# LIA-DiTella/DiffUDF

Hardware: AMD Instinct MI355X
Metric: train points/sec (SIREN fwd+∇x+Eikonal loss+bwd), 256×8 net, 100k pts (higher is better)
Workload: dtype f32

## Files before the change

### diffudf_amd/_lib.py

```python
import ctypes
import os

_HERE = os.path.dirname(os.path.abspath(__file__))
LIB_PATH = os.environ.get("DUDF_LIB") or os.path.join(_HERE, "libdudf_hip.so")

LOSS_S1, LOSS_S2, LOSS_SIREN = 0, 1, 2

_ERRORS = {
    -1: "DUDF_E_BADCFG: unsupported network (kernel width in {32,64,128,256,512} — hip_ops pads narrower / unequal layers —, n_in=3, n_out=1)",
    -2: "DUDF_E_WORKSPACE: workspace too small or misaligned",
    -3: "DUDF_E_BADMODE",
    -4: "DUDF_E_UNSUPPORTED: this configuration has no HIP path; there is deliberately no CPU fallback",
}


class NetCfg(ctypes.Structure):
    _fields_ = [("n_in", ctypes.c_int32), ("n_hidden_layers", ctypes.c_int32),
                ("hidden", ctypes.c_int32), ("w0", ctypes.c_float), ("ww", ctypes.c_float)]


class DudfError(RuntimeError):
    pass


# ... 65 lines not shown
                                            ctypes.c_size_t, _P]),
    "dudf_adam_step": (ctypes.c_int, [_P, _P, _P, _P, ctypes.c_int64, ctypes.c_double, ctypes.c_double,
                                      ctypes.c_double, ctypes.c_double, ctypes.c_int64, ctypes.c_double, _P]),
    "dudf_adam_schedule": (ctypes.c_int, [_DBL, ctypes.c_int64, ctypes.c_int64, ctypes.c_double, ctypes.c_double, _P]),
    "dudf_adam_step_scheduled": (ctypes.c_int, [_P, _P, _P, _P, ctypes.c_int64, ctypes.c_double, ctypes.c_double, ctypes.c_double,
                                                _P, ctypes.c_int64, _P, ctypes.c_double, _P]),
    "dudf_sample_batch_at": (ctypes.c_int, [_P, ctypes.c_int64, _P, _P, ctypes.c_int64, ctypes.c_int64, ctypes.c_int64,
                                            ctypes.c_int64, ctypes.c_uint64, _P, ctypes.c_int, ctypes.c_int, _P, _P, _P, _P]),
    "dudf_sample_batch": (ctypes.c_int, [_P, ctypes.c_int64, _P, _P, ctypes.c_int64, ctypes.c_int64, ctypes.c_int64,
                                         ctypes.c_int64, ctypes.c_uint64, ctypes.c_uint64, ctypes.c_int, ctypes.c_int,
                                         _P, _P, _P, _P]),
    "dudf_capudf_workspace_bytes": (ctypes.c_size_t, [ctypes.c_int64]),
    "dudf_capudf_count": (ctypes.c_int, [_P, _P, ctypes.c_int64, ctypes.c_double, _P, _P, ctypes.c_size_t, _P]),
    "dudf_capudf_emit": (ctypes.c_int, [_P, _P, ctypes.c_int64, ctypes.c_double, _P, _P, _P, _P, ctypes.c_size_t, _P]),
    "dudf_profile_enable": (ctypes.c_int, [ctypes.c_int]),
    "dudf_split_mode": (ctypes.c_int, []),
    "dudf_profile_dump": (ctypes.c_int, [ctypes.c_char_p, ctypes.c_size_t]),
    "dudf_profile_clocks": (ctypes.c_int, [ctypes.c_char_p, ctypes.c_size_t]),
    "dudf_profile_products": (ctypes.c_int, [ctypes.c_char_p, ctypes.c_size_t]),
    "dudf_set_wgrad_max_workgroups": (ctypes.c_int, [ctypes.c_int]),
    "dudf_debug_read_stash": (ctypes.c_int, [_CFG, ctypes.c_int, ctypes.c_int, ctypes.c_int, ctypes.c_int64,
                                             ctypes.c_int64, _P, _P, ctypes.c_size_t, _P]),
    "dudf_debug_stash_layout": (ctypes.c_int, [_CFG, ctypes.c_int64, ctypes.c_int64, ctypes.POINTER(ctypes.c_int64)]),
    "dudf_debug_kernel_choice": (ctypes.c_int, [_CFG, ctypes.c_int64, ctypes.c_int64, ctypes.c_int, ctypes.c_int, ctypes.c_char_p, ctypes.c_size_t]),
    "dudf_stash_mode": (ctypes.c_int, [_CFG, ctypes.c_int64, ctypes.c_int64]),
    "dudf_set_option": (ctypes.c_int, [ctypes.c_char_p, ctypes.c_int]),
    "dudf_get_option": (ctypes.c_int, [ctypes.c_char_p, ctypes.POINTER(ctypes.c_int)]),
    "dudf_reset_options": (ctypes.c_int, []),
    "dudf_abi_version": (ctypes.c_int, []),
}
ABI_VERSION = 8


def load():
    global _lib
    if _lib is not None:
        return _lib
    if not os.path.exists(LIB_PATH):
        raise DudfError(f"{LIB_PATH} not found: build it with `python -c 'import __graft_entry__ as g; g.build()'` "
                        "(hipcc --offload-arch=gfx950). There is no CPU fallback for the HIP path.")
    lib = ctypes.CDLL(LIB_PATH)
    try:
        lib.dudf_abi_version.restype = ctypes.c_int
        abi = int(lib.dudf_abi_version())
    except AttributeError:
        abi = None
# ... 22 lines not shown
```

### diffudf_amd/csrc/dudf_api.hip

```cpp
#include "dudf_internal.h"
#include <stdio.h>
#include <stdlib.h>
#include <string.h>
#include <vector>

namespace {
struct ProfRec { int slot; hipEvent_t e0, e1; };
bool g_prof_on = false;
std::vector<ProfRec> g_prof_recs;
std::vector<hipEvent_t> g_prof_pool;
hipEvent_t g_prof_open[PROF_NSLOTS];
const char* kProfNames[PROF_NSLOTS] = {"pack", "sweep_fwd", "sweep_rev", "sweep_adj_fwd", "sweep_adj_rev",
                                       "wgrad_hidden", "wgrad_small", "loss_fwd", "loss_bwd", "adam", "other"};
unsigned long long* g_prof_clk = nullptr;
hipEvent_t prof_event() {
    if (!g_prof_pool.empty()) { hipEvent_t e = g_prof_pool.back(); g_prof_pool.pop_back(); return e; }
    hipEvent_t e; (void)hipEventCreate(&e); return e;
}
}

namespace { int g_products[PROF_NSLOTS] = {0}; }
void dudf_note_products(int slot, int products) { if (slot >= 0 && slot < PROF_NSLOTS) g_products[slot] = products; }

unsigned long long* dudf_prof_clk(int slot) { return (g_prof_on && g_prof_clk) ? g_prof_clk + 2 * slot : nullptr; }
// ... 803 lines not shown
    if (layer < 0 || layer >= c.lo.L || channel < 0 || channel > 3) return DUDF_E_BADCFG;
    const DudfLayout& lo = c.lo;
    const int64_t offs[8] = {lo.ws_S, lo.ws_C, lo.ws_Q, lo.ws_E, lo.ws_A, lo.ws_Z, lo.ws_R, lo.ws_ZS};
    if (which < 0 || which > 7) return DUDF_E_BADMODE;
    const bool sqaz = which == 0 || which == 2 || which == 4 || which == 5;
    const int b24 = which == 7 ? 0 : which == 1 ? ((lo.p24 & 4) ? 2 : 0) : sqaz ? ((lo.p24 & 1) ? 3 : 0) : ((lo.p24 & 2) ? 1 : 0);
    const int fxi = which == 0 ? 0 : which == 2 ? 1 : which == 4 ? 2 : 3;
    return dudf_launch_read_stash(lo, c.ws + offs[which], layer, channel, out, c.st, which == 1, b24,
                                  b24 == 3 ? c.ws + lo.ws_fx[fxi] : nullptr);
}

int dudf_debug_stash_layout(const dudf_net_cfg* cfg, int64_t n, int64_t n_hess, int64_t* out) {
    DudfLayout lo;
    int rc = dudf_make_layout(cfg, n, n_hess, &lo);
    if (rc) return rc;
    if (!out) return DUDF_E_BADCFG;
    const int64_t offs[8] = {lo.ws_S, lo.ws_C, lo.ws_Q, lo.ws_E, lo.ws_A, lo.ws_Z, lo.ws_R, lo.ws_ZS};
    for (int i = 0; i < 8; ++i) out[i] = offs[i] * (int64_t)sizeof(float);
    out[8] = lo.np * 16;
    out[9] = lo.stash_layer * (int64_t)sizeof(float);
    return 0;
}

int dudf_debug_kernel_choice(const dudf_net_cfg* cfg, int64_t n, int64_t n_hess, int which, int flags, char* name, size_t name_len) {
    DudfLayout lo;
    int rc = dudf_make_layout(cfg, n, n_hess, &lo, (flags & 16) != 0);
    if (rc) return rc;
    if (!name || name_len == 0) return DUDF_E_BADCFG;
    name[0] = 0;
    SweepChoice c;
    if (which == DUDF_CHOICE_WGRAD) {
        c = dudf_choose_wgrad(WgradRequest{lo.H, lo.L, lo.p24 & 1, lo.np}, dudf_options());
    } else {
        const SweepRequest r = {which & 15, lo.H, lo.L, flags & 1, (flags >> 1) & 1, (flags >> 2) & 1, (flags >> 3) & 1, split_mask(), lo.p24,
                                lo.ws_ebound != lo.ws_amax, lo.ws_zbound != lo.ws_amax};
        c = (which & DUDF_CHOICE_PAIR) ? dudf_choose_pair(r, dudf_options()) : dudf_choose_sweep(r, dudf_options());
    }
    if (c.status == 0 && dudf_choice_name(c, name, name_len) >= (int)name_len) return DUDF_E_WORKSPACE;
    return c.status;
}

int dudf_stash_mode(const dudf_net_cfg* cfg, int64_t n, int64_t n_hess) {
    DudfLayout lo;
    if (dudf_make_layout(cfg, n, n_hess, &lo)) return -1;
    return lo.p24;
}
// ... 3 lines not shown
```

### diffudf_amd/csrc/dudf_internal.h

```cpp
#pragma once
#include <hip/hip_runtime.h>
#include <stdint.h>
#include <stdlib.h>
#include "../../include/dudf_hip.h"
#include "dudf_variants.h"

typedef float f32x4 __attribute__((ext_vector_type(4)));
typedef float f32x16 __attribute__((ext_vector_type(16)));
typedef float f32x2 __attribute__((ext_vector_type(2)));
typedef unsigned u32x4 __attribute__((ext_vector_type(4)));
typedef __bf16 bf16x8 __attribute__((ext_vector_type(8)));
typedef __bf16 bf16x2 __attribute__((ext_vector_type(2)));
typedef _Float16 f16x8 __attribute__((ext_vector_type(8)));
typedef _Float16 f16x2 __attribute__((ext_vector_type(2)));

__device__ __forceinline__ unsigned cvt_pk(f32x2 v) {
    return __builtin_bit_cast(unsigned, __builtin_convertvector(v, bf16x2));
}
__device__ __forceinline__ f32x2 unpack(unsigned p) {
    return f32x2{__builtin_bit_cast(float, p << 16), __builtin_bit_cast(float, p & 0xffff0000u)};
}

#define DUDF_TILE_PTS 64
#define DUDF_COL_PAD 128
#define DUDF_NACC 16

struct DudfLayout {
    int H, L;
    float rho;
    int p24;
    float w0;
    int64_t n, n_h;
    int64_t ncol_h, ncol_n;
    int64_t ncols;
    int64_t np;
    int64_t off_w1, off_b1, off_hid, hid_stride, off_wo, off_bo, n_theta;
    int64_t ws_w1b, ws_b1s, ws_w1t16, ws_wt, ws_wimg, ws_wimg16, ws_wsc, ws_amax, ws_ebound, ws_zbound, ws_x4, ws_y, ws_g, ws_ybar, ws_gbar;
    int64_t ws_S, ws_C, ws_ZS, ws_Q, ws_R, ws_E, ws_A, ws_Z, ws_acc;
    int64_t ws_fx[4];
    int64_t stash_layer;
    size_t total_bytes;
};

DudfOptions dudf_options();

static inline int dudf_make_layout(const dudf_net_cfg* cfg, int64_t n, int64_t n_h, DudfLayout* lo, int query_only = 0) {
    if (!cfg || cfg->n_in != 3 || cfg->n_hidden_layers < 1) return DUDF_E_BADCFG;
    const int H = cfg->hidden, L = cfg->n_hidden_layers;
    if (!(H == 32 || H == 64 || H == 128 || H == 256 || H == 512)) return DUDF_E_BADCFG;
    if (n < 0 || n_h < 0 || n_h > n) return DUDF_E_BADCFG;
    if (!(cfg->w0 > 0.f) || cfg->ww < 0.f) return DUDF_E_BADCFG;
    const float ww = cfg->ww > 0.f ? cfg->ww : cfg->w0;
    lo->H = H; lo->L = L; lo->w0 = ww; lo->rho = cfg->w0 / ww;
    lo->n = n; lo->n_h = n_h;
    lo->p24 = query_only ? 0 : dudf_stash_p24_enabled(H, L, dudf_options());
    auto pad = [](int64_t c) { return (c + DUDF_COL_PAD - 1) / DUDF_COL_PAD * DUDF_COL_PAD; };
    lo->ncol_h = pad(4 * n_h);
    lo->ncol_n = pad(n - n_h);
    lo->np = lo->ncol_h + lo->ncol_n;
    if (lo->np == 0) { lo->ncol_n = DUDF_COL_PAD; lo->np = DUDF_COL_PAD; }
    lo->ncols = lo->np;
    if (lo->np % 2048 == 0) lo->np += 32;
    if (lo->np * 1024 >= (1ll << 32)) lo->p24 = 0;
// ... 11 lines not shown
    lo->ws_wimg16 = take((int64_t)(L - 1) * H * H * 2);
    lo->ws_wsc = take(2 * (int64_t)(L > 1 ? L - 1 : 1));
    lo->ws_amax = take(4 * (int64_t)L);
    lo->ws_ebound = query_only ? lo->ws_amax : take((int64_t)L * lo->np);
    lo->ws_zbound = (n_h == 0) ? lo->ws_amax : take((int64_t)L * lo->ncol_h);
    lo->ws_x4 = take(4 * lo->np);
    lo->ws_y = take(lo->np); lo->ws_g = take(4 * lo->np);
    lo->ws_ybar = take(lo->np); lo->ws_gbar = take(4 * lo->np);
    lo->stash_layer = (int64_t)H * lo->np;
    const int64_t stash = (int64_t)L * lo->stash_layer;
    const int64_t stash_b = (lo->p24 & 1) ? stash / 4 * 3 : stash;
    const int64_t stash_r = (lo->p24 & 2) ? stash / 4 * 3 : stash;
    const int64_t stash_c = (lo->p24 & 4) ? stash / 4 * 3 : stash;
    lo->ws_S = take(stash_b); lo->ws_C = take(stash_c);
    lo->ws_ZS = n_h > 0 ? take(stash) : lo->ws_S;
    if (query_only) {
        lo->ws_Q = lo->ws_R = lo->ws_E = lo->ws_A = lo->ws_Z = lo->ws_S;
    } else {
        lo->ws_Q = take(stash_b); lo->ws_R = take(stash_r); lo->ws_E = take(stash_r); lo->ws_A = take(stash_b);
        lo->ws_Z = take(stash_b);
    }
    for (int i = 0; i < 4; ++i) lo->ws_fx[i] = (lo->p24 & 1) ? take((int64_t)L * lo->np) : lo->ws_amax;
    lo->ws_acc = take(2 * DUDF_NACC);
    lo->total_bytes = (size_t)o * sizeof(float);
    return 0;
}

#if defined(__HIP_DEVICE_COMPILE__)
#define DUDF_NO_PK __attribute__((target("no-packed-fp32-ops")))
#else
#define DUDF_NO_PK
#endif

struct SweepArgs {
    const float* theta; const float* w1b; const float* b1s; const float* w1t16; const float* wt;
    const char* wimg_f; const char* wimg_t;
    const char* wimg16_f; const char* wimg16_t;
    const float* wsc;
    unsigned* amax;
    float* ebound;
    float* zbound;
    int64_t nch;
    unsigned long long* clk;
    int split;
    const float* x4;
    float* y; float* g;
// ... 105 lines not shown
```

### diffudf_amd/csrc/dudf_prep.hip

```cpp
#include "dudf_sweep16.h"

namespace {

template <int H>
__device__ __forceinline__ void pack_bf16_body(const float* __restrict__ theta, char* __restrict__ img_f,
                                               char* __restrict__ img_t, int nhid, int64_t off_hid,
                                               int64_t hid_stride, int64_t block, int64_t nblocks) {
    using G = GeoB<H>;
    const int64_t total = (int64_t)2 * nhid * G::NKB * G::NT * 64;
    for (int64_t idx = block * 256 + threadIdx.x; idx < total; idx += nblocks * 256) {
        int64_t v = idx;
        const int lane = (int)(v & 63); v >>= 6;
        const int T = (int)(v % G::NT); v /= G::NT;
        const int kb = (int)(v % G::NKB); v /= G::NKB;
        const int j = (int)(v % nhid); v /= nhid;
        const int dir = (int)v;
        const int m = lane & 15, g = lane >> 4;
        const int row = 16 * T + m;
        const float* W = theta + off_hid + (int64_t)j * hid_stride;
        f32x4 e0, e1;
#pragma unroll
        for (int e = 0; e < 4; ++e) {
            const int f0 = 32 * kb + 4 * g + e, f1 = f0 + 16;
            e0[e] = dir == 0 ? W[(int64_t)row * H + f0] : W[(int64_t)f0 * H + row];
// ... 53 lines not shown
            e1[e] = sc * (dir == 0 ? W[(int64_t)row * H + f1] : W[(int64_t)f1 * H + row]);
        }
        u32x4 h, l;
        split8h(e0, e1, h, l);
        char* base = (dir == 0 ? img_f : img_t) + (size_t)j * G::IMGB + (size_t)kb * G::CHUNKB + (size_t)T * 2 * G::FRAG + lane * 16;
        *reinterpret_cast<u32x4*>(base) = h;
        *reinterpret_cast<u32x4*>(base + G::FRAG) = l;
    }
}
template <int H>
__global__ __launch_bounds__(256) void pack_f16_kernel(const float* __restrict__ theta, char* __restrict__ img_f,
                                                       char* __restrict__ img_t, float* __restrict__ wsc, int nhid,
                                                       int64_t off_hid, int64_t hid_stride) {
    pack_f16_body<H>(theta, img_f, img_t, wsc, nhid, off_hid, hid_stride, blockIdx.y, blockIdx.x, gridDim.x);
}

struct PrepArgs {
    const float* theta; const float* x;
    float *w1b, *b1s, *w1t16, *wt, *x4, *wsc;
    float rho;
    char *img16_f, *img16_t, *img_f, *img_t;
    unsigned* zero; int nzero;
    unsigned* zero2; int nzero2;
    int L, nsub;
    int64_t off_hid, hid_stride, n, n_h, ncol_h, np;
    int nb_f16, nb_bf16, nb_x4, nb_thin, nb_wt;
};
template <int H>
__global__ __launch_bounds__(256) void prep_kernel(PrepArgs a) {
    int b = blockIdx.x;
    const int nhid = a.L - 1;
    if (b < a.nb_f16) { pack_f16_body<H>(a.theta, a.img16_f, a.img16_t, a.wsc, nhid, a.off_hid, a.hid_stride, b / a.nsub, b % a.nsub, a.nsub); return; }
    b -= a.nb_f16;
    if (b < a.nb_bf16) { pack_bf16_body<H>(a.theta, a.img_f, a.img_t, nhid, a.off_hid, a.hid_stride, b, a.nb_bf16); return; }
    b -= a.nb_bf16;
    if (b < a.nb_x4) {
        for (int64_t c = (int64_t)b * 256 + threadIdx.x; c < a.np; c += (int64_t)a.nb_x4 * 256) {
            f32x4 v = {0, 0, 0, 0};
            if (c < a.ncol_h) {
                const int64_t p = c >> 2; const int ch = (int)(c & 3);
                if (p < a.n_h) {
                    if (ch == 0) v = f32x4{a.x[p * 3], a.x[p * 3 + 1], a.x[p * 3 + 2], 1.f};
                    else v[ch - 1] = 1.f;
                }
            } else {
                const int64_t p = a.n_h + (c - a.ncol_h);
// ... 4 lines not shown
        return;
    }
    b -= a.nb_x4;
    if (b < a.nb_thin) {
        const int n_thin = 16 * H > a.L * H ? 16 * H : a.L * H;
        for (int gid = b * 256 + threadIdx.x; gid < n_thin; gid += a.nb_thin * 256) {
            if (gid < 4 * H) {
                const int f = gid / 4, k = gid % 4;
                a.w1b[gid] = a.rho * (k < 3 ? a.theta[f * 3 + k] : a.theta[3 * H + f]);
                if (k == 3) a.b1s[f] = a.rho * a.theta[3 * H + f];
            }
            if (gid >= H && gid < a.L * H) {
                const int layer = gid / H, f = gid % H;
                a.b1s[gid] = a.theta[a.off_hid + (int64_t)(layer - 1) * a.hid_stride + (int64_t)H * H + f];
            }
            if (gid < 16 * H) {
                const int r = gid / H, f = gid % H;
                a.w1t16[gid] = r < 3 ? a.rho * a.theta[f * 3 + r] : 0.f;
            }
        }
        if (b == 0) {
            for (int i = threadIdx.x; i < a.nzero; i += 256) a.zero[i] = 0u;
            for (int i = threadIdx.x; i < a.nzero2; i += 256) a.zero2[i] = 0u;
        }
        return;
    }
    b -= a.nb_thin;
    {
        const int64_t n_wt = (int64_t)nhid * H * H;
        for (int64_t gid = (int64_t)b * 256 + threadIdx.x; gid < n_wt; gid += (int64_t)a.nb_wt * 256) {
            const int64_t j = gid / ((int64_t)H * H), rem = gid % ((int64_t)H * H);
            const int i = (int)(rem / H), o = (int)(rem % H);
            a.wt[gid] = a.theta[a.off_hid + j * a.hid_stride + (int64_t)o * H + i];
        }
    }
}

template <int H>
int pack_b(const DudfLayout& lo, const float* theta, float* ws, hipStream_t st) {
    using G = GeoB<H>;
    char* img_f = reinterpret_cast<char*>(ws + lo.ws_wimg);
    char* img_t = img_f + (size_t)(lo.L - 1) * G::IMGB;
    const int64_t total = (int64_t)2 * (lo.L - 1) * G::NKB * G::NT * 64;
    hipLaunchKernelGGL(pack_bf16_kernel<H>, dim3((unsigned)((total + 255) / 256)), dim3(256), 0, st, theta, img_f, img_t,
                       lo.L - 1, lo.off_hid, lo.hid_stride);
    if (dudf_split_fp16()) {
        using G1 = GeoB<H, 1>;
        char* i16_f = reinterpret_cast<char*>(ws + lo.ws_wimg16);
        char* i16_t = i16_f + (size_t)(lo.L - 1) * G1::IMGB;
        hipLaunchKernelGGL(pack_f16_kernel<H>, dim3(H >= 256 ? 16 : 4, lo.L - 1), dim3(256), 0, st, theta, i16_f, i16_t,
                           ws + lo.ws_wsc, lo.L - 1, lo.off_hid, lo.hid_stride);
    }
    return (int)hipGetLastError();
}

template <int H>
int prep_b(const DudfLayout& lo, const float* theta, const float* x, float* ws, int need, hipStream_t st) {
    PrepArgs a;
    a.theta = theta; a.x = x;
    a.w1b = ws + lo.ws_w1b; a.b1s = ws + lo.ws_b1s; a.rho = lo.rho; a.w1t16 = ws + lo.ws_w1t16; a.wt = ws + lo.ws_wt; a.x4 = ws + lo.ws_x4; a.wsc = ws + lo.ws_wsc;
    a.img_f = reinterpret_cast<char*>(ws + lo.ws_wimg); a.img_t = a.img_f + (size_t)(lo.L - 1) * GeoB<H>::IMGB;
    a.img16_f = reinterpret_cast<char*>(ws + lo.ws_wimg16); a.img16_t = a.img16_f + (size_t)(lo.L - 1) * GeoB<H, 1>::IMGB;
    a.zero = reinterpret_cast<unsigned*>(ws + lo.ws_acc); a.nzero = 2 * DUDF_NACC;
    a.zero2 = reinterpret_cast<unsigned*>(ws + lo.ws_amax); a.nzero2 = 4 * lo.L;
    a.L = lo.L; a.off_hid = lo.off_hid; a.hid_stride = lo.hid_stride;
    a.n = lo.n; a.n_h = lo.n_h; a.ncol_h = lo.ncol_h; a.np = lo.np;
    const int nhid = lo.L - 1;
    a.nsub = H >= 256 ? 16 : 4;
    a.nb_f16 = (dudf_split_fp16() && nhid > 0) ? nhid * a.nsub : 0;
    a.nb_bf16 = ((need & 1) && nhid > 0) ? (int)(((int64_t)2 * nhid * GeoB<H>::NKB * GeoB<H>::NT * 64 + 255) / 256) : 0;
    a.nb_x4 = x ? (int)((lo.np + 255) / 256 < 1024 ? (lo.np + 255) / 256 : 1024) : 0;
    a.nb_thin = 2;
    a.nb_wt = ((need & 2) && nhid > 0) ? (int)(((int64_t)nhid * H * H + 255) / 256 < 2048 ? ((int64_t)nhid * H * H + 255) / 256 : 2048) : 0;
    const int grid = a.nb_f16 + a.nb_bf16 + a.nb_x4 + a.nb_thin + a.nb_wt;
    hipLaunchKernelGGL(prep_kernel<H>, dim3(grid), dim3(256), 0, st, a);
    return (int)hipGetLastError();
}
}

int dudf_launch_prep(const DudfLayout& lo, const float* theta, const float* x, float* ws, int need, hipStream_t st) {
    DudfProfScope prof(PROF_PACK, st);
    if (lo.H == 256) return prep_b<256>(lo, theta, x, ws, need, st);
    if (lo.H == 128) return prep_b<128>(lo, theta, x, ws, need, st);
    if (lo.H == 512) return prep_b<512>(lo, theta, x, ws, need, st);
    return DUDF_E_UNSUPPORTED;
}

// ... 9 lines not shown
```

### diffudf_amd/csrc/dudf_variants.h

```cpp
#pragma once
#include <stddef.h>
#include <stdint.h>
#include <stdio.h>
#include <utility>
#include "../../include/dudf_hip.h"

enum { SWEEP_FWD = 0, SWEEP_REV = 1, SWEEP_ADJ_FWD = 2, SWEEP_ADJ_REV = 3,
       SWEEP_FWD_H = 4, SWEEP_REV_H = 5, SWEEP_ADJ_FWD_H = 6, SWEEP_ADJ_REV_H = 7,
       SWEEP_FWD_J = 8 };

struct DudfOptions {
    int deterministic, split, split_quads, sweep_family, stash, wgrad_family, wgrad_tr, pair_launch, wgrad_max_workgroups, wgrad_buffers;
};
inline int dudf_split_mask(const DudfOptions& o) { return o.split ? (15 | (o.split_quads ? 32 : 0)) : 0; }

struct DudfVariant { int sw, fl, p24; };
constexpr DudfVariant kF32Variants[] = {{0, 3, 0}, {1, 1, 0}, {1, 0, 0}, {2, 0, 0}, {3, 1, 0}, {3, 0, 0},
                                        {4, 1, 0}, {5, 1, 0}, {5, 0, 0}, {6, 0, 0}, {7, 0, 0}, {8, 0, 0}};
constexpr DudfVariant kSweepVariants[] = {{0, 3, 1}, {0, 2, 0}, {0, 0, 0}, {1, 1, 1}, {1, 0, 0}, {2, 0, 1}, {3, 1, 1}, {3, 0, 1},
                                          {4, 1, 1}, {4, 0, 0}, {5, 1, 1}, {5, 0, 0}, {6, 0, 1}, {7, 0, 1}, {8, 0, 0}};
constexpr DudfVariant kWideVariants[] = {{0, 3, 1}, {0, 1, 0}, {1, 1, 1}, {1, 0, 0}, {2, 0, 1}, {3, 1, 1}, {3, 0, 1},
                                         {4, 1, 1}, {5, 1, 1}, {5, 0, 0}, {6, 0, 1}, {7, 0, 1}, {8, 0, 0}};
constexpr DudfVariant kPairVariants[] = {{0, 3, 1}, {1, 1, 1}, {2, 0, 1}, {3, 1, 1}};
constexpr int dudf_pair_flq(int sw) { return sw <= SWEEP_REV ? 1 : 0; }
// ... 164 lines not shown
        return c;
    };
    if (!(H == 32 || H == 64 || H == 128 || H == 256)) return dudf_no_choice(DUDF_E_BADCFG);
    if (r.p24 && (o.wgrad_family != 0 || H != 256)) return dudf_no_choice(DUDF_E_UNSUPPORTED);
    if (o.wgrad_family == 1) return pick(DUDF_FAM_WG_F32, 0, 1, 4 * (size_t)(H / 4) * 33 * 4 * sizeof(float));
    const size_t lds_wave = (size_t)4 * 2 * (H / 4) * 16 * 4 * sizeof(float);
    if (H != 256 || o.wgrad_family == 2 || (int64_t)(r.H / 4) * r.np * 16 >= (1ll << 32)) return pick(DUDF_FAM_WG_BF16, 0, 6, lds_wave);
    const bool f16 = o.split && r.L <= kMaxAmaxLayers;
    const size_t lds_t = (size_t)(2 * 2 * 16 * 576);
    if (r.p24) {
        if (!(f16 && ntz == 1)) return dudf_no_choice(DUDF_E_UNSUPPORTED);
        return o.wgrad_buffers == 4 ? pick(DUDF_FAM_WG_F16P24, 25, 3, 4 * lds_t + 512) : pick(DUDF_FAM_WG_F16P24, 9, 3, 3 * lds_t + 512);
    }
    if (o.wgrad_tr && f16 && ntz == 1 && !o.deterministic) return pick(DUDF_FAM_WG_F16TR, 9, 3, 3 * lds_t + 512);
    const size_t lds_piece = (size_t)2 * (H / 32) * 2 * (32 * 16 + 16);
    if (f16) {
        SweepChoice c = pick(DUDF_FAM_WG_F16P, 9, 3, 3 * 2 * lds_piece + 512);
        c.remap = ntz == 4 && !o.deterministic;
        return c;
    }
    return pick(DUDF_FAM_WG_BF16P, 9, 6, 3 * 3 * lds_piece + 512);
}

inline int dudf_stash_p24_enabled(int H, int L, const DudfOptions& o) {
    int want = o.stash & 7;
    if (want != 0 && want != 6 && want != 7) want = 6;
    if (!(o.sweep_family && o.split && (dudf_split_mask(o) & 47) == 47)) want = 0;
    if (o.wgrad_family != 0) want &= 6;
    if (H == 256 && L >= 2 && L <= 32) return want;
    if (H == 512 && L >= 2) return want & 6;
    return 0;
}

inline int dudf_choice_name(const SweepChoice& c, char* buf, size_t n) {
    const char* np = c.no_pk ? "_np" : "";
    switch (c.family) {
        case DUDF_FAM_F32: return snprintf(buf, n, "sweep_kernel<%d,%d,%d>", c.H, c.sw, c.fl);
        case DUDF_FAM_BF16: return snprintf(buf, n, "sweep_bf16%s_kernel<%d,%d,%d>", np, c.H, c.sw, c.fl);
        case DUDF_FAM_F16:
            return snprintf(buf, n, "sweep_f16%s_kernel<%d,%d,%d>", np, c.H, c.sw, c.fl);
        case DUDF_FAM_F16R: return snprintf(buf, n, "sweep_f16r%s_kernel<%d,%d,%d>", np, c.H, c.sw, c.fl);
        case DUDF_FAM_F16P: return snprintf(buf, n, "sweep_f16p%s_kernel<%d,%d,%d>", np, c.H, c.sw, c.fl);
        case DUDF_FAM_W: return snprintf(buf, n, "sweep_w_kernel<%d,%d>", c.sw, c.fl);
        case DUDF_FAM_W16: return snprintf(buf, n, "sweep_w16_kernel<%d,%d>", c.sw, c.fl);
        case DUDF_FAM_W16R: return snprintf(buf, n, "sweep_w16r_kernel<%d,%d>", c.sw, c.fl);
        case DUDF_FAM_PAIR: return snprintf(buf, n, "sweep_pair_kernel<256,%d,%d,%d,%d,%d,%d>", c.swq, c.flq, c.sw, c.fl, c.spq, c.p24);
// ... 10 lines not shown
```

### diffudf_amd/csrc/dudf_wgrad.hip

```cpp
#include "dudf_internal.h"
#include <stdlib.h>
#include <string.h>
#include <type_traits>

namespace {

template <int H> struct WG;
template <> struct WG<256> { static constexpr int WO = 4, WI = 2, MT = 2, NTL = 4; };
template <> struct WG<128> { static constexpr int WO = 4, WI = 2, MT = 1, NTL = 2; };
template <> struct WG<64>  { static constexpr int WO = 2, WI = 2, MT = 1, NTL = 1; };
template <> struct WG<32>  { static constexpr int WO = 1, WI = 1, MT = 1, NTL = 1; };

constexpr int KT = 32;
constexpr int KTP = 33;

struct WgradArgs {
    const float *Q, *A, *Z, *S;
    int64_t ncol_h;
    float* dtheta;
    int64_t np, stash_layer, off_hid, hid_stride;
    int steps_total;
    int L;
    int have_g;
    int j0, nj;
// ... 783 lines not shown
    if (clk_on && tid == 0) {
        a.clk[0] = __builtin_amdgcn_s_memtime() - clk_t0;
        a.clk[1] = __builtin_amdgcn_s_memrealtime() - clk_r0;
    }
}
template <int VAR> constexpr int wg_buffers() { static_assert(VAR == 9 || VAR == 25, "VAR 9: three image buffers, 25: four"); return VAR == 25 ? 4 : 3; }
template <int H, int VAR>
__global__ __launch_bounds__(64 * WG<H>::WO * WG<H>::WI) DUDF_NO_PK void wgrad_hidden_bf16p_kernel(WgradArgs a) {
    wgrad_hidden_bf16p_body<H, wg_buffers<VAR>()>(a);
}
template <int H, int VAR>
__global__ __launch_bounds__(64 * WG<H>::WO * WG<H>::WI) DUDF_NO_PK void wgrad_hidden_f16p_kernel(WgradArgs a) {
    wgrad_hidden_bf16p_body<H, wg_buffers<VAR>(), 1>(a);
}
template <int H, int VAR>
__global__ __launch_bounds__(64 * WG<H>::WO * WG<H>::WI) DUDF_NO_PK void wgrad_hidden_f16tr_kernel(WgradArgs a) {
    wgrad_hidden_bf16p_body<H, wg_buffers<VAR>(), 1, 2>(a);
}
template <int H, int VAR>
__global__ __launch_bounds__(64 * WG<H>::WO * WG<H>::WI) DUDF_NO_PK void wgrad_hidden_f16p24_kernel(WgradArgs a) {
    wgrad_hidden_bf16p_body<H, wg_buffers<VAR>(), 1, 1>(a);
}

#ifndef DUDF_WGSMALL_P24_PTS
#define DUDF_WGSMALL_P24_PTS 4096
#endif
struct WgradSmallArgs {
    const float *Q, *A, *Z, *S;
    const float *x4, *gbar, *ybar;
    float* dtheta;
    int64_t np, ncols, stash_layer, off_wo, off_bo;
    int H, L, have_g;
    int pts_per_block;
    float rho;
    const float *fxS, *fxQ, *fxA, *fxZ;
};

__device__ __forceinline__ float wave_sum(float v) {
#pragma unroll
    for (int o = 32; o > 0; o >>= 1) v += __shfl_xor(v, o);
    return v;
}

__device__ __forceinline__ void wgrad_small_body(const WgradSmallArgs& a) {
    const int lane = threadIdx.x & 63, wave = threadIdx.x >> 6;
    const int FQ = a.H / 4;
    const int64_t p0 = (int64_t)blockIdx.x * a.pts_per_block;
    const int64_t p1 = (p0 + a.pts_per_block < a.ncols) ? p0 + a.pts_per_block : a.ncols;
    const float* Q0 = a.Q;
    const float* Z0 = a.Z;
    const float* AL = a.A + (int64_t)(a.L - 1) * a.stash_layer;
    const float* SL = a.S + (int64_t)(a.L - 1) * a.stash_layer;
    const int fq_per = (FQ + gridDim.y - 1) / gridDim.y;
    const int fq_lo = blockIdx.y * fq_per, fq_hi = (fq_lo + fq_per < FQ) ? fq_lo + fq_per : FQ;
    for (int fq = fq_lo + wave; fq < fq_hi; fq += 4) {
        float w1[4][4], wo[4];
#pragma unroll
        for (int c = 0; c < 4; ++c) { wo[c] = 0.f; w1[c][0] = w1[c][1] = w1[c][2] = w1[c][3] = 0.f; }
// ... 20 lines not shown
#pragma unroll
        for (int c = 0; c < 4; ++c) {
            const int f = 4 * fq + c;
#pragma unroll
            for (int d = 0; d < 4; ++d) {
                const float v = wave_sum(w1[c][d]);
                if (lane == 0) atomicAdd(d < 3 ? a.dtheta + f * 3 + d : a.dtheta + 3 * a.H + f, a.rho * v);
            }
            const float vo = wave_sum(wo[c]);
            if (lane == 0) atomicAdd(a.dtheta + a.off_wo + f, vo);
        }
    }
    if (wave == 0 && blockIdx.y == 0) {
        float s = 0.f;
        for (int64_t p = p0 + lane; p < p1; p += 64) s += a.ybar[p];
        s = wave_sum(s);
        if (lane == 0) atomicAdd(a.dtheta + a.off_bo, s);
    }
}
__global__ __launch_bounds__(256) DUDF_NO_PK void wgrad_small_kernel(WgradSmallArgs a) { wgrad_small_body(a); }

__device__ __forceinline__ f32x4 small_unpack24(const unsigned* g, const float sc) {
    typedef unsigned u3_t __attribute__((ext_vector_type(3)));
    const u3_t d = __builtin_nontemporal_load(reinterpret_cast<const u3_t*>(g));
    const unsigned d0 = d.x, d1 = d.y, d2 = d.z;
    const unsigned m = 0x00ffffffu, two = 0x40000000u;
    const unsigned y = __builtin_amdgcn_perm(d1, d0, 0x0c0c0703u);
    const unsigned t3 = __builtin_amdgcn_perm(d2, y, 0x0c070100u) | two;
    const float m3 = -3.0f * sc;
    return f32x4{__builtin_fmaf(__uint_as_float((d0 & m) | two), sc, m3), __builtin_fmaf(__uint_as_float((d1 & m) | two), sc, m3),
                 __builtin_fmaf(__uint_as_float((d2 & m) | two), sc, m3), __builtin_fmaf(__uint_as_float(t3), sc, m3)};
}
__global__ __launch_bounds__(256) DUDF_NO_PK void wgrad_small_p24_kernel(WgradSmallArgs a) {
    const int lane = threadIdx.x & 63, wave = threadIdx.x >> 6;
    const int q = lane >> 4, li = lane & 15, T = blockIdx.y;
    const int64_t ng = a.np >> 4;
    const int64_t g0 = (int64_t)blockIdx.x * (a.pts_per_block >> 4);
    const int64_t gend = (a.ncols + 15) >> 4;
    const int64_t g1 = g0 + (a.pts_per_block >> 4) < gend ? g0 + (a.pts_per_block >> 4) : gend;
    const int64_t lbytes = a.stash_layer * 3;
    auto tile = [&](const float* arr, int layer) { return reinterpret_cast<const char*>(arr) + (int64_t)layer * lbytes + (int64_t)T * ng * 768 + lane * 12; };
    const char* Q0 = tile(a.Q, 0); const char* Z0 = tile(a.Z, 0);
    const char* AL = tile(a.A, a.L - 1); const char* SL = tile(a.S, a.L - 1);
    float w1[4][4], wo[4];
#pragma unroll
    for (int c = 0; c < 4; ++c) { wo[c] = 0.f; w1[c][0] = w1[c][1] = w1[c][2] = w1[c][3] = 0.f; }
    float sy = 0.f;
    const int nwave = (int)(blockDim.x >> 6);
#pragma unroll 4
    for (int64_t g = g0 + wave; g < g1; g += nwave) {
        const int64_t p = g * 16 + li;
        const f32x4 z = small_unpack24(reinterpret_cast<const unsigned*>(Z0 + g * 768), a.fxZ[p]);
        const f32x4 sl = small_unpack24(reinterpret_cast<const unsigned*>(SL + g * 768), a.fxS[(int64_t)(a.L - 1) * a.np + p]);
        const f32x4 xv = *reinterpret_cast<const f32x4*>(a.x4 + p * 4);
        const float yb = a.ybar[p];
        f32x4 qv = {0, 0, 0, 0}, al = {0, 0, 0, 0}, gb = {0, 0, 0, 0};
        if (a.have_g) {
            qv = small_unpack24(reinterpret_cast<const unsigned*>(Q0 + g * 768), a.fxQ[p]);
            al = small_unpack24(reinterpret_cast<const unsigned*>(AL + g * 768), a.fxA[(int64_t)(a.L - 1) * a.np + p]);
            gb = *reinterpret_cast<const f32x4*>(a.gbar + p * 4);
        }
        sy += yb;
#pragma unroll
        for (int c = 0; c < 4; ++c) {
#pragma unroll
            for (int d = 0; d < 4; ++d) w1[c][d] += qv[c] * gb[d] + z[c] * xv[d];
            wo[c] += al[c] * xv[3] + yb * sl[c];
        }
    }
    auto sum16 = [](float v) { v += __shfl_xor(v, 1); v += __shfl_xor(v, 2); v += __shfl_xor(v, 4); v += __shfl_xor(v, 8); return v; };
    __shared__ float red[4][4][21];
#pragma unroll
    for (int c = 0; c < 4; ++c) {
#pragma unroll
        for (int d = 0; d < 4; ++d) {
            const float v = sum16(w1[c][d]);
            if (li == 0) red[wave][q][c * 4 + d] = v;
        }
        const float vo = sum16(wo[c]);
        if (li == 0) red[wave][q][16 + c] = vo;
    }
    {
        const float v = sum16(sy);
        if (li == 0) red[wave][q][20] = v;
    }
    __syncthreads();
    for (int t = threadIdx.x; t < 81; t += blockDim.x) {
        if (t < 80) {
            const int qq = t / 20, k = t % 20;
            float v = 0.f;
            for (int w = 0; w < nwave; ++w) v += red[w][qq][k];
            if (k < 16) {
                const int c = k >> 2, d = k & 3, f = 16 * T + 4 * qq + c;
                atomicAdd(d < 3 ? a.dtheta + f * 3 + d : a.dtheta + 3 * a.H + f, a.rho * v);
            } else {
                atomicAdd(a.dtheta + a.off_wo + 16 * T + 4 * qq + (k - 16), v);
            }
        } else if (T == 0) {
            float v = 0.f;
            for (int w = 0; w < nwave; ++w) v += red[w][0][20];
            atomicAdd(a.dtheta + a.off_bo, v);
        }
    }
}

static_assert(KTP == 33 && NRING == 4 && KB == 16, "dudf_choose_wgrad: LDS sizes");
template <int H>
int launch_hidden(const SweepChoice& c, const WgradArgs& a, hipStream_t st) {
    using W = WG<H>;
    const int tz = a.Hs / H, ntz = tz * tz;
    int nsplit = dudf_wgrad_max_workgroups() / (a.nj * ntz);
    if (nsplit > a.steps_total) nsplit = a.steps_total;
    if (nsplit < 1 || dudf_deterministic()) nsplit = 1;
    const dim3 grid(a.nj, nsplit, ntz), block(64 * W::WO * W::WI);
    if (c.family == DUDF_FAM_WG_F32) return dudf_launch_kernel<&wgrad_hidden_kernel<H>>(grid, block, c.lds, c.lds_max, st, a);
    if (c.family == DUDF_FAM_WG_BF16) return dudf_launch_kernel<&wgrad_hidden_bf16_kernel<H>>(grid, block, c.lds, c.lds_max, st, a);
    if constexpr (H == 256) {
        if (c.family == DUDF_FAM_WG_F16P24 && c.fl == 25) return dudf_launch_kernel<&wgrad_hidden_f16p24_kernel<H, 25>>(grid, block, c.lds, c.lds_max, st, a);
        if (c.family == DUDF_FAM_WG_F16P24) return dudf_launch_kernel<&wgrad_hidden_f16p24_kernel<H, 9>>(grid, block, c.lds, c.lds_max, st, a);
        if (c.family == DUDF_FAM_WG_F16TR) return dudf_launch_kernel<&wgrad_hidden_f16tr_kernel<H, 9>>(grid, block, c.lds, c.lds_max, st, a);
        if (c.family == DUDF_FAM_WG_BF16P) return dudf_launch_kernel<&wgrad_hidden_bf16p_kernel<H, 9>>(grid, block, c.lds, c.lds_max, st, a);
        if (c.family == DUDF_FAM_WG_F16P && c.remap) {
            WgradArgs b = a;
            b.remap_nsplit = nsplit;
            return dudf_launch_kernel<&wgrad_hidden_f16p_kernel<H, 9>>(dim3(((a.nj * nsplit + 7) / 8) * 32), block, c.lds, c.lds_max, st, b);
        }
// ... 25 lines not shown
        DudfProfScope prof(PROF_WGRAD_HIDDEN, st);
        const SweepChoice c = dudf_choose_wgrad(WgradRequest{lo.H, lo.L, a.p24, lo.np}, dudf_options());
        if (c.status) return c.status;
        dudf_note_products(PROF_WGRAD_HIDDEN, c.products);
        switch (c.H) {
            case 32: rc = launch_hidden<32>(c, a, st); break;
            case 64: rc = launch_hidden<64>(c, a, st); break;
            case 128: rc = launch_hidden<128>(c, a, st); break;
            default: rc = launch_hidden<256>(c, a, st); break;
        }
    }
    if (rc) return rc;
    if (!(layer_begin <= 0 || layer_end >= lo.L + 1)) return 0;
    WgradSmallArgs s;
    s.Q = a.Q; s.A = a.A; s.Z = a.Z; s.S = a.S; s.x4 = ws + lo.ws_x4; s.gbar = ws + lo.ws_gbar; s.ybar = ws + lo.ws_ybar;
    s.dtheta = dtheta; s.np = lo.np; s.ncols = lo.ncols; s.stash_layer = lo.stash_layer;
    s.off_wo = lo.off_wo; s.off_bo = lo.off_bo; s.H = lo.H; s.L = lo.L; s.have_g = have_g; s.rho = lo.rho;
    s.fxS = a.fxS; s.fxQ = a.fxQ; s.fxA = a.fxA; s.fxZ = a.fxZ;
    s.pts_per_block = dudf_deterministic() ? (int)lo.ncols : 4096;
    const int grid = (int)((lo.ncols + s.pts_per_block - 1) / s.pts_per_block);
    DudfProfScope prof(PROF_WGRAD_SMALL, st);
    const int fqn = lo.H / 4;
    const int gy = fqn >= 64 ? 16 : (fqn >= 4 ? fqn / 4 : 1);
    if (lo.p24 & 1) {
        if (!dudf_deterministic()) {
            s.pts_per_block = DUDF_WGSMALL_P24_PTS;
            const int64_t want = (lo.ncols / 30 + 255) / 256 * 256;
            if (want < s.pts_per_block) s.pts_per_block = want < 512 ? 512 : (int)want;
        }
        s.pts_per_block = (s.pts_per_block + 15) / 16 * 16;
        hipLaunchKernelGGL(wgrad_small_p24_kernel, dim3((unsigned)((lo.ncols + s.pts_per_block - 1) / s.pts_per_block), lo.H / 16),
                           dim3(dudf_deterministic() ? 64 : 256), 0, st, s);
        return (int)hipGetLastError();
    }
    hipLaunchKernelGGL(wgrad_small_kernel, dim3(grid, gy), dim3(256), 0, st, s);
    return (int)hipGetLastError();
}
```

### include/dudf_hip.h

```cpp
#ifndef DUDF_HIP_H
#define DUDF_HIP_H
#include <stddef.h>
#include <stdint.h>

#ifdef __cplusplus
extern "C" {
#endif

#define DUDF_ABI_VERSION 8
int dudf_abi_version(void);

#define DUDF_E_BADCFG   (-1)
#define DUDF_E_WORKSPACE (-2)
#define DUDF_E_BADMODE  (-3)
#define DUDF_E_UNSUPPORTED (-4)

#define DUDF_LOSS_S1    0
#define DUDF_LOSS_S2    1
#define DUDF_LOSS_SIREN 2

typedef struct dudf_net_cfg {
    int32_t n_in;
    int32_t n_hidden_layers;
    int32_t hidden;
// ... 120 lines not shown
int dudf_weight_gradient(const dudf_net_cfg* cfg, int64_t n_local, int64_t n_hess, int have_gradient_terms, int layer_begin,
                         int layer_end, float* dtheta, int accumulate, void* workspace, size_t workspace_bytes, void* stream);

int dudf_fields_forward(const dudf_net_cfg* cfg, const float* theta, const float* x, int64_t n,
                        float* out_f, float* out_g, void* workspace, size_t workspace_bytes, void* stream);
int dudf_fields_backward(const dudf_net_cfg* cfg, const float* theta, const float* x, int64_t n,
                         const float* ybar, const float* gbar, float* dtheta, int accumulate,
                         void* workspace, size_t workspace_bytes, void* stream);

int dudf_adam_step(float* theta, const float* dtheta, float* exp_avg, float* exp_avg_sq, int64_t n,
                   double lr, double beta1, double beta2, double eps, int64_t step, double grad_scale,
                   void* stream);

int dudf_adam_schedule(const double* lr, int64_t n_steps, int64_t first_step, double beta1, double beta2, float* out);
int dudf_adam_step_scheduled(float* theta, const float* dtheta, float* exp_avg, float* exp_avg_sq, int64_t n,
                             double beta1, double beta2, double eps, const float* sched, int64_t n_rows, const int64_t* row,
                             double grad_scale, void* stream);

int dudf_debug_read_stash(const dudf_net_cfg* cfg, int which, int layer, int channel, int64_t n, int64_t n_hess,
                          float* out, void* workspace, size_t workspace_bytes, void* stream);

int dudf_debug_stash_layout(const dudf_net_cfg* cfg, int64_t n, int64_t n_hess, int64_t* out);

#define DUDF_CHOICE_PAIR 16
#define DUDF_CHOICE_WGRAD (-1)
int dudf_debug_kernel_choice(const dudf_net_cfg* cfg, int64_t n, int64_t n_hess, int which, int flags, char* name, size_t name_len);

int dudf_stash_mode(const dudf_net_cfg* cfg, int64_t n, int64_t n_hess);

int dudf_sample_batch(const float* tri, int64_t n_tri, const float* pc_pos, const float* pc_nrm, int64_t n_pc,
                      int64_t n_on, int64_t n_far, int64_t n_near, uint64_t seed, uint64_t step, int rank, int world,
                      float* x, float* normals, float* sdf, void* stream);
int dudf_sample_batch_at(const float* tri, int64_t n_tri, const float* pc_pos, const float* pc_nrm, int64_t n_pc,
                         int64_t n_on, int64_t n_far, int64_t n_near, uint64_t seed, const int64_t* step_dev, int rank, int world,
                         float* x, float* normals, float* sdf, void* stream);

int dudf_profile_enable(int on);
int dudf_profile_dump(char* buf, size_t buflen);
int dudf_profile_clocks(char* buf, size_t buflen);
int dudf_profile_products(char* buf, size_t buflen);

int dudf_set_option(const char* name, int value);
int dudf_get_option(const char* name, int* value);
int dudf_reset_options(void);
int dudf_set_wgrad_max_workgroups(int n);

// ... 10 lines not shown
```

Before: 39.25 million.

## Replace wgrad_small p24 global atomics with two-level last-block reduction

```diff
diff --git a/diffudf_amd/_lib.py b/diffudf_amd/_lib.py
--- a/diffudf_amd/_lib.py
+++ b/diffudf_amd/_lib.py
@@ -111,6 +111,7 @@
     "dudf_debug_read_stash": (ctypes.c_int, [_CFG, ctypes.c_int, ctypes.c_int, ctypes.c_int, ctypes.c_int64,
                                              ctypes.c_int64, _P, _P, ctypes.c_size_t, _P]),
     "dudf_debug_stash_layout": (ctypes.c_int, [_CFG, ctypes.c_int64, ctypes.c_int64, ctypes.POINTER(ctypes.c_int64)]),
+    "dudf_debug_thin_layout": (ctypes.c_int, [_CFG, ctypes.c_int64, ctypes.c_int64, ctypes.POINTER(ctypes.c_int64)]),
     "dudf_debug_kernel_choice": (ctypes.c_int, [_CFG, ctypes.c_int64, ctypes.c_int64, ctypes.c_int, ctypes.c_int, ctypes.c_char_p, ctypes.c_size_t]),
     "dudf_stash_mode": (ctypes.c_int, [_CFG, ctypes.c_int64, ctypes.c_int64]),
     "dudf_set_option": (ctypes.c_int, [ctypes.c_char_p, ctypes.c_int]),
diff --git a/diffudf_amd/csrc/dudf_api.hip b/diffudf_amd/csrc/dudf_api.hip
--- a/diffudf_amd/csrc/dudf_api.hip
+++ b/diffudf_amd/csrc/dudf_api.hip
@@ -849,6 +849,18 @@
     return 0;
 }
 
+int dudf_debug_thin_layout(const dudf_net_cfg* cfg, int64_t n, int64_t n_hess, int64_t* out) {
+    DudfLayout lo;
+    int rc = dudf_make_layout(cfg, n, n_hess, &lo);
+    if (rc) return rc;
+    if (!out) return DUDF_E_BADCFG;
+    const ThinChoice tc = dudf_choose_thin(lo.H, lo.p24, lo.ncols);
+    out[0] = (lo.thin_floats ? lo.ws_thin : (int64_t)(lo.total_bytes / sizeof(float))) * (int64_t)sizeof(float);
+    out[1] = (int64_t)lo.total_bytes - out[0];
+    out[2] = tc.cols_per_block; out[3] = tc.blocks;
+    return 0;
+}
+
 int dudf_debug_kernel_choice(const dudf_net_cfg* cfg, int64_t n, int64_t n_hess, int which, int flags, char* name, size_t name_len) {
     DudfLayout lo;
     int rc = dudf_make_layout(cfg, n, n_hess, &lo, (flags & 16) != 0);
diff --git a/diffudf_amd/csrc/dudf_internal.h b/diffudf_amd/csrc/dudf_internal.h
--- a/diffudf_amd/csrc/dudf_internal.h
+++ b/diffudf_amd/csrc/dudf_internal.h
@@ -39,6 +39,7 @@
     int64_t ws_S, ws_C, ws_ZS, ws_Q, ws_R, ws_E, ws_A, ws_Z, ws_acc;
     int64_t ws_fx[4];
     int64_t stash_layer;
+    int64_t ws_thin, thin_floats;
     size_t total_bytes;
 };
 
@@ -96,6 +97,8 @@
     }
     for (int i = 0; i < 4; ++i) lo->ws_fx[i] = (lo->p24 & 1) ? take((int64_t)L * lo->np) : lo->ws_amax;
     lo->ws_acc = take(2 * DUDF_NACC);
+    lo->thin_floats = query_only ? 0 : dudf_choose_thin(H, lo->p24, lo->ncols).scratch_floats;
+    lo->ws_thin = lo->thin_floats ? take(lo->thin_floats) : lo->ws_amax;
     lo->total_bytes = (size_t)o * sizeof(float);
     return 0;
 }
diff --git a/diffudf_amd/csrc/dudf_prep.hip b/diffudf_amd/csrc/dudf_prep.hip
--- a/diffudf_amd/csrc/dudf_prep.hip
+++ b/diffudf_amd/csrc/dudf_prep.hip
@@ -99,6 +99,7 @@
     char *img16_f, *img16_t, *img_f, *img_t;
     unsigned* zero; int nzero;
     unsigned* zero2; int nzero2;
+    unsigned* zero3; int nzero3;
     int L, nsub;
     int64_t off_hid, hid_stride, n, n_h, ncol_h, np;
     int nb_f16, nb_bf16, nb_x4, nb_thin, nb_wt;
@@ -149,6 +150,7 @@
         if (b == 0) {
             for (int i = threadIdx.x; i < a.nzero; i += 256) a.zero[i] = 0u;
             for (int i = threadIdx.x; i < a.nzero2; i += 256) a.zero2[i] = 0u;
+            for (int i = threadIdx.x; i < a.nzero3; i += 256) a.zero3[i] = 0u;
         }
         return;
     }
@@ -190,6 +192,7 @@
     a.img16_f = reinterpret_cast<char*>(ws + lo.ws_wimg16); a.img16_t = a.img16_f + (size_t)(lo.L - 1) * GeoB<H, 1>::IMGB;
     a.zero = reinterpret_cast<unsigned*>(ws + lo.ws_acc); a.nzero = 2 * DUDF_NACC;
     a.zero2 = reinterpret_cast<unsigned*>(ws + lo.ws_amax); a.nzero2 = 4 * lo.L;
+    a.zero3 = reinterpret_cast<unsigned*>(ws + lo.ws_thin); a.nzero3 = lo.thin_floats ? kThinTicketWords : 0;
     a.L = lo.L; a.off_hid = lo.off_hid; a.hid_stride = lo.hid_stride;
     a.n = lo.n; a.n_h = lo.n_h; a.ncol_h = lo.ncol_h; a.np = lo.np;
     const int nhid = lo.L - 1;
diff --git a/diffudf_amd/csrc/dudf_variants.h b/diffudf_amd/csrc/dudf_variants.h
--- a/diffudf_amd/csrc/dudf_variants.h
+++ b/diffudf_amd/csrc/dudf_variants.h
@@ -210,6 +210,21 @@
     return pick(DUDF_FAM_WG_BF16P, 9, 6, 3 * 3 * lds_piece + 512);
 }
 
+constexpr int kThinTicketWords = 64;
+constexpr int kThinPartStride = 84;
+constexpr int kThinMaxBlocks = 64;
+struct ThinChoice { int two_level, cols_per_block, blocks, tiles; int64_t scratch_floats; };
+inline ThinChoice dudf_choose_thin(int H, int p24, int64_t ncols) {
+    ThinChoice c = {};
+    if (!(p24 & 1)) return c;
+    int64_t cols = ((ncols + kThinMaxBlocks - 1) / kThinMaxBlocks + 15) / 16 * 16;
+    if (cols < 512) cols = 512;
+    c.two_level = 1; c.cols_per_block = (int)cols; c.blocks = (int)((ncols + cols - 1) / cols); c.tiles = H / 16;
+    if (c.blocks < 1) c.blocks = 1;
+    c.scratch_floats = kThinTicketWords + (int64_t)c.blocks * c.tiles * kThinPartStride;
+    return c;
+}
+
 inline int dudf_stash_p24_enabled(int H, int L, const DudfOptions& o) {
     int want = o.stash & 7;
     if (want != 0 && want != 6 && want != 7) want = 6;
diff --git a/diffudf_amd/csrc/dudf_wgrad.hip b/diffudf_amd/csrc/dudf_wgrad.hip
--- a/diffudf_amd/csrc/dudf_wgrad.hip
+++ b/diffudf_amd/csrc/dudf_wgrad.hip
@@ -829,9 +829,6 @@
     wgrad_hidden_bf16p_body<H, wg_buffers<VAR>(), 1, 1>(a);
 }
 
-#ifndef DUDF_WGSMALL_P24_PTS
-#define DUDF_WGSMALL_P24_PTS 4096
-#endif
 struct WgradSmallArgs {
     const float *Q, *A, *Z, *S;
     const float *x4, *gbar, *ybar;
@@ -841,6 +838,7 @@
     int pts_per_block;
     float rho;
     const float *fxS, *fxQ, *fxA, *fxZ;
+    float* part; unsigned* tick;
 };
 
 __device__ __forceinline__ float wave_sum(float v) {
@@ -907,7 +905,7 @@
 
 __device__ __forceinline__ f32x4 small_unpack24(const unsigned* g, const float sc) {
     typedef unsigned u3_t __attribute__((ext_vector_type(3)));
-    const u3_t d = __builtin_nontemporal_load(reinterpret_cast<const u3_t*>(g));
+    const u3_t d = *reinterpret_cast<const u3_t*>(g);
     const unsigned d0 = d.x, d1 = d.y, d2 = d.z;
     const unsigned m = 0x00ffffffu, two = 0x40000000u;
     const unsigned y = __builtin_amdgcn_perm(d1, d0, 0x0c0c0703u);
@@ -916,7 +914,7 @@
     return f32x4{__builtin_fmaf(__uint_as_float((d0 & m) | two), sc, m3), __builtin_fmaf(__uint_as_float((d1 & m) | two), sc, m3),
                  __builtin_fmaf(__uint_as_float((d2 & m) | two), sc, m3), __builtin_fmaf(__uint_as_float(t3), sc, m3)};
 }
-__global__ __launch_bounds__(256) DUDF_NO_PK void wgrad_small_p24_kernel(WgradSmallArgs a) {
+__global__ __launch_bounds__(256) void wgrad_small_p24_kernel(WgradSmallArgs a) {
     const int lane = threadIdx.x & 63, wave = threadIdx.x >> 6;
     const int q = lane >> 4, li = lane & 15, T = blockIdx.y;
     const int64_t ng = a.np >> 4;
@@ -931,9 +929,8 @@
 #pragma unroll
     for (int c = 0; c < 4; ++c) { wo[c] = 0.f; w1[c][0] = w1[c][1] = w1[c][2] = w1[c][3] = 0.f; }
     float sy = 0.f;
-    const int nwave = (int)(blockDim.x >> 6);
-#pragma unroll 4
-    for (int64_t g = g0 + wave; g < g1; g += nwave) {
+#pragma unroll 2
+    for (int64_t g = g0 + wave; g < g1; g += 4) {
         const int64_t p = g * 16 + li;
         const f32x4 z = small_unpack24(reinterpret_cast<const unsigned*>(Z0 + g * 768), a.fxZ[p]);
         const f32x4 sl = small_unpack24(reinterpret_cast<const unsigned*>(SL + g * 768), a.fxS[(int64_t)(a.L - 1) * a.np + p]);
@@ -955,6 +952,8 @@
     }
     auto sum16 = [](float v) { v += __shfl_xor(v, 1); v += __shfl_xor(v, 2); v += __shfl_xor(v, 4); v += __shfl_xor(v, 8); return v; };
     __shared__ float red[4][4][21];
+    __shared__ float fin[4][kThinPartStride];
+    __shared__ unsigned last;
 #pragma unroll
     for (int c = 0; c < 4; ++c) {
 #pragma unroll
@@ -970,23 +969,42 @@
         if (li == 0) red[wave][q][20] = v;
     }
     __syncthreads();
-    for (int t = threadIdx.x; t < 81; t += blockDim.x) {
+    const int t = threadIdx.x;
+    const int nrows = (int)gridDim.x, ntiles = (int)gridDim.y;
+    if (t < 81) {
+        const int qq = t < 80 ? t / 20 : 0, k = t < 80 ? t % 20 : 20;
+        const float v = ((red[0][qq][k] + red[1][qq][k]) + red[2][qq][k]) + red[3][qq][k];
+        __hip_atomic_store(a.part + ((int64_t)blockIdx.x * ntiles + T) * kThinPartStride + t, v, __ATOMIC_RELAXED, __HIP_MEMORY_SCOPE_AGENT);
+    }
+    __threadfence();
+    __syncthreads();
+    if (t == 0) last = (atomicAdd(a.tick + T, 1u) == (unsigned)nrows - 1u) ? 1u : 0u;
+    __syncthreads();
+    if (!last) return;
+    __threadfence();
+    for (int e = lane; e < 81; e += 64) {
+        float v = 0.f;
+        for (int r = wave; r < nrows; r += 4)
+            v += __hip_atomic_load(a.part + ((int64_t)r * ntiles + T) * kThinPartStride + e, __ATOMIC_RELAXED, __HIP_MEMORY_SCOPE_AGENT);
+        fin[wave][e] = v;
+    }
+    __syncthreads();
+    if (t < 81) {
+        const float v = ((fin[0][t] + fin[1][t]) + fin[2][t]) + fin[3][t];
         if (t < 80) {
             const int qq = t / 20, k = t % 20;
-            float v = 0.f;
-            for (int w = 0; w < nwave; ++w) v += red[w][qq][k];
             if (k < 16) {
                 const int c = k >> 2, d = k & 3, f = 16 * T + 4 * qq + c;
-                atomicAdd(d < 3 ? a.dtheta + f * 3 + d : a.dtheta + 3 * a.H + f, a.rho * v);
+                float* o = d < 3 ? a.dtheta + f * 3 + d : a.dtheta + 3 * a.H + f;
+                *o += a.rho * v;
             } else {
-                atomicAdd(a.dtheta + a.off_wo + 16 * T + 4 * qq + (k - 16), v);
+                a.dtheta[a.off_wo + 16 * T + 4 * qq + (k - 16)] += v;
             }
         } else if (T == 0) {
-            float v = 0.f;
-            for (int w = 0; w < nwave; ++w) v += red[w][0][20];
-            atomicAdd(a.dtheta + a.off_bo, v);
-        }
-    }
+            a.dtheta[a.off_bo] += v;
+        }
+    }
+    if (t == 0) atomicExch(a.tick + T, 0u);
 }
 
 static_assert(KTP == 33 && NRING == 4 && KB == 16, "dudf_choose_wgrad: LDS sizes");
@@ -1058,15 +1076,13 @@
     DudfProfScope prof(PROF_WGRAD_SMALL, st);
     const int fqn = lo.H / 4;
     const int gy = fqn >= 64 ? 16 : (fqn >= 4 ? fqn / 4 : 1);
-    if (lo.p24 & 1) {
-        if (!dudf_deterministic()) {
-            s.pts_per_block = DUDF_WGSMALL_P24_PTS;
-            const int64_t want = (lo.ncols / 30 + 255) / 256 * 256;
-            if (want < s.pts_per_block) s.pts_per_block = want < 512 ? 512 : (int)want;
-        }
-        s.pts_per_block = (s.pts_per_block + 15) / 16 * 16;
-        hipLaunchKernelGGL(wgrad_small_p24_kernel, dim3((unsigned)((lo.ncols + s.pts_per_block - 1) / s.pts_per_block), lo.H / 16),
-                           dim3(dudf_deterministic() ? 64 : 256), 0, st, s);
+    s.part = nullptr; s.tick = nullptr;
+    const ThinChoice tc = dudf_choose_thin(lo.H, lo.p24, lo.ncols);
+    if (tc.two_level) {
+        if (tc.scratch_floats != lo.thin_floats) return DUDF_E_WORKSPACE;
+        s.pts_per_block = tc.cols_per_block;
+        s.tick = reinterpret_cast<unsigned*>(ws + lo.ws_thin); s.part = ws + lo.ws_thin + kThinTicketWords;
+        hipLaunchKernelGGL(wgrad_small_p24_kernel, dim3((unsigned)tc.blocks, (unsigned)tc.tiles), dim3(256), 0, st, s);
         return (int)hipGetLastError();
     }
     hipLaunchKernelGGL(wgrad_small_kernel, dim3(grid, gy), dim3(256), 0, st, s);
diff --git a/include/dudf_hip.h b/include/dudf_hip.h
--- a/include/dudf_hip.h
+++ b/include/dudf_hip.h
@@ -166,6 +166,8 @@
 
 int dudf_debug_stash_layout(const dudf_net_cfg* cfg, int64_t n, int64_t n_hess, int64_t* out);
 
+int dudf_debug_thin_layout(const dudf_net_cfg* cfg, int64_t n, int64_t n_hess, int64_t* out);
+
 #define DUDF_CHOICE_PAIR 16
 #define DUDF_CHOICE_WGRAD (-1)
 int dudf_debug_kernel_choice(const dudf_net_cfg* cfg, int64_t n, int64_t n_hess, int which, int flags, char* name, size_t name_len);
```

After: 37.74 million. -3.8%, worse.
